# ikramanop/aligner

Hardware: AMD Instinct MI355X
Metric: GCUPS (DP cell updates/s), fill + traceback, inputs resident in HBM (higher is better)
Workload: dtype int32; 1 GPU; C5: 100000 protein pairs, lengths iid U[200,2000], core local (SimpleLocalAligner), BLOSUM62, del 11 / ext 2, seed 0xA11C0005; pairs=100000, cells=121325988939, pairs_ok_rank0=100000, pairs_repaired_or_refilled_rank0=65570

## Files before the change

aligner_amd/csrc/aln_fast.h:

```cpp
#pragma once

__device__ __forceinline__ int v_max3(int a, int b, int c)
{
    int d;
    asm("v_max3_i32 %0, %1, %2, %3" : "=v"(d) : "v"(a), "v"(b), "v"(c));
    return d;
}
__device__ __forceinline__ int v_tform(int key)
{
    int d;
    asm("v_and_or_b32 %0, %1, -4, 2" : "=v"(d) : "v"(key));
    return d;
}
__device__ __forceinline__ int v_add3_m1(int a, int b)
{
    int d;
    asm("v_add3_u32 %0, %1, %2, -1" : "=v"(d) : "v"(a), "v"(b));
    return d;
}
__device__ __forceinline__ int v_pack11(int t, int kterm)
{
    int d;
    asm("v_lshl_add_u32 %0, %1, 11, %2" : "=v"(d) : "v"(t), "s"(kterm));
    return d;
}
#define ALN_CELL_ASM(BYTE)                                                                                    \
    asm("v_add_u32_sdwa %0, %8, sext(%9) dst_sel:DWORD dst_unused:UNUSED_PAD src0_sel:DWORD src1_sel:" BYTE "\n\t" \
        "v_add_u32 %1, %5, %7\n\t"                                                                            \
        "v_add3_u32 %2, %6, %7, -1\n\t"                                                                       \
        "v_max3_i32 %3, %1, %2, %0\n\t"                                                                       \
        "v_and_or_b32 %4, %3, -4, 2"                                                                          \
        : "=&v"(c), "=&v"(a), "=&v"(b), "=&v"(key), "=v"(nt)                                                  \
        : "v"(top), "v"(left), "v"(negp), "v"(diag), "v"(pw))
template <int B>
__device__ __forceinline__ void v_cell(int top, int left, int negp, int diag, uint32_t pw, int &key, int &nt)
{
    int a, b, c;
    if constexpr (B == 0) ALN_CELL_ASM("BYTE_0");
    else if constexpr (B == 1) ALN_CELL_ASM("BYTE_1");
    else if constexpr (B == 2) ALN_CELL_ASM("BYTE_2");
    else ALN_CELL_ASM("BYTE_3");
}
#undef ALN_CELL_ASM

template <int RP> struct ProfWordP;
template <> struct ProfWordP<8> { using T = uint2; };
template <> struct ProfWordP<4> { using T = uint32_t; };
template <> struct ProfWordP<2> { using T = uint16_t; };
template <> struct ProfWordP<1> { using T = uint8_t; };
template <int R> struct ProfWord {
    static constexpr int RP = R > 4 ? 8 : R > 2 ? 4 : R;
    using T = typename ProfWordP<RP>::T;
};

template <int R>
__device__ __forceinline__ uint32_t prof_word(const typename ProfWord<R>::T &pw, int r)
{
    if constexpr (R > 4) return r < 4 ? pw.x : pw.y;
    else return (uint32_t)pw;
}
template <int R>
__device__ __forceinline__ int prof_byte(const typename ProfWord<R>::T &pw, int r)
{
    if constexpr (R > 4) return (int)(int8_t)(((r < 4 ? pw.x : pw.y) >> (8 * (r & 3))) & 0xff);
    else return (int)(int8_t)(((uint32_t)pw >> (8 * r)) & 0xff);
}

__device__ __forceinline__ int shr1_i(int old, int v) { return __builtin_amdgcn_update_dpp(old, v, 0x138, 0xf, 0xf, false); }

typedef __attribute__((address_space(3))) uint8_t aln_lds_u8;
typedef __attribute__((address_space(3))) int aln_lds_i32;
__device__ __forceinline__ void qring_put(uint32_t ring, uint32_t c, uint32_t code)
{
    const uint32_t i = c & 127u;
    *(aln_lds_u8 *)(uintptr_t)(ring + i) = (uint8_t)code;
    if (i < 64u) *(aln_lds_u8 *)(uintptr_t)(ring + 128u + i) = (uint8_t)code;
}
__device__ __forceinline__ int qring_get(uint32_t addr) { return (int)*(const aln_lds_u8 *)(uintptr_t)addr; }
__device__ __forceinline__ void bring_put(uint32_t addr, int v) { *(aln_lds_i32 *)(uintptr_t)addr = v; }
__device__ __forceinline__ int bring_get(uint32_t addr) { return *(const aln_lds_i32 *)(uintptr_t)addr; }

__device__ __forceinline__ void granule_store(uint32_t *p, int v)
{
    __hip_atomic_store(p, (uint32_t)v, __ATOMIC_RELAXED, __HIP_MEMORY_SCOPE_AGENT);
}
__device__ __forceinline__ uint32_t granule_load(const uint32_t *p)
{
    return __hip_atomic_load(p, __ATOMIC_RELAXED, __HIP_MEMORY_SCOPE_AGENT);
}

#include "aln_single_unit.inc"

#define ALN_RING 4096u

struct FastIn {
    int lane;
    uint32_t N, M;
    const uint8_t *q, *t;
    const int *S;
    uint32_t cols;
    uint8_t *prof;
    uint32_t qring;
    uint32_t brow_ring;
    int nd4, ne4;
    uint32_t *dirw;
    unsigned long long *brow_in, *brow_out;
    uint8_t *advice, *zrow;
    int *ckpt;
    bool hazard;
    bool adv_any;
    bool store_dirs;
    bool wt_dirs;
    bool pwm;
    const uint32_t *pwm_words;
    uint32_t ck_stop;
    int ck_mode;
    uint32_t last_flip;
    uint16_t *qo_pad;
    int *bring;
    const uint32_t *gin;
    uint32_t *gout;
    uint32_t lds_scratch;
    uint32_t *ring_in, *ring_out;
    uint32_t *abort_flag;
    uint32_t strip_rows, strip_q16;
    uint32_t tag_base;
    uint32_t fair;
    uint32_t ck_last;
};

struct FastOut {
    int bv;
    uint32_t by, bx;
    int corner;
    bool repaired, brow_bad, aborted;
    uint32_t ck_slot;
    uint32_t c_out;
};

template <int SEM>
__device__ __forceinline__ bool better_i(int v, uint32_t y, uint32_t x, int bv, uint32_t by, uint32_t bx)
{
    if (v > bv) return true;
    if (v < bv) return false;
    if (SEM == ALN_CORE_LOCAL) return y < by || (y == by && x < bx);
    return x > bx || (x == bx && y > by);
}

__device__ __forceinline__ uint32_t uniform32(uint32_t v) { return (uint32_t)__builtin_amdgcn_readfirstlane((int)v); }
__device__ __forceinline__ uint64_t uniform64(uint64_t v)
{
    const uint32_t lo = (uint32_t)__builtin_amdgcn_readfirstlane((int)(uint32_t)v);
    const uint32_t hi = (uint32_t)__builtin_amdgcn_readfirstlane((int)(uint32_t)(v >> 32));
    return ((uint64_t)hi << 32) | lo;
}
__device__ __forceinline__ uint64_t uniform64(const void *p) { return uniform64((uint64_t)(uintptr_t)p); }

template <int SEM, int R, bool SINGLE, bool FIRST, bool LAST, bool PWM = false>
struct FastStrip {
    static constexpr int SPB = (int)aln_spb(R);
    static constexpr int RP = ProfWord<R>::RP;
    static constexpr uint32_t CHUNK = (2048u / (4u * SPB)) * (4u * SPB);
    static constexpr uint32_t STRIP_ROWS = SINGLE ? 64u * R : (uint32_t)ALN_STRIP_ROWS;
    static constexpr bool LOCAL = (SEM == ALN_CORE_LOCAL || SEM == ALN_LEGACY_LOCAL);
    static constexpr bool QRING = !SINGLE && !PWM;
    static constexpr bool BRING = QRING && !FIRST;
    static constexpr int QSHIFT = RP == 8 ? 9 : RP == 4 ? 8 : RP == 2 ? 7 : 6;
    using PW = typename ProfWord<R>::T;
    const FastIn in;
    const uint32_t strip;
    static constexpr bool last = LAST;
    const int lane;
    const uint32_t N;
    uint32_t lb, rb, yb;
    uint32_t chunk0;
    uint32_t cchg;
    bool zsel_on, brow_bad, aborted;
    int Tl[R], rbv[R];
    int hdiag, bottom, qoff, inchunk, qchunk, outq;
    uint32_t advchunk, dw;
    PW pw;
    const uint8_t *prow;
    uint32_t qaddr;
    uint32_t baddr;

    const uint8_t *qo_lane;
    int *bring;
    int qv, top0v;
    uint32_t gpre;
    static constexpr bool GLOBAL_ASM = (SEM == ALN_CORE_GLOBAL);
    static constexpr bool ASMPATH = SINGLE && (SEM == ALN_CORE_LOCAL || SEM == ALN_CORE_GLOBAL) && (R == 1 || R == 2) && !(FIRST && LAST);
    int twov;
    PW pw1;
    uint32_t qv2, qv3, gA, gB;
    bool insteady;
    bool ring_staged;

    __device__ __forceinline__ FastStrip(const FastIn &i, uint32_t s)
        : in(i), strip(s), lane(i.lane), N(i.N), cchg(0), brow_bad(false), aborted(false) {}

    uint32_t psel_lo, psel_hi;
    __device__ __forceinline__ PW pwm_select(uint32_t w4) const
    {
        if constexpr (R > 4) return make_uint2(__builtin_amdgcn_perm(w4, w4, psel_lo), __builtin_amdgcn_perm(w4, w4, psel_hi));
        else return (PW)__builtin_amdgcn_perm(w4, w4, psel_lo);
    }

    __device__ __forceinline__ int fetch_above(uint32_t xi)
    {
        const uint32_t want = in.tag_base | (strip - 1u);
        const unsigned long long *p = in.brow_in + xi + 1;
        unsigned long long g = 0;
        uint32_t spins = 0;
        for (;;) {
            if (xi < N) g = __hip_atomic_load(p, __ATOMIC_RELAXED, __HIP_MEMORY_SCOPE_AGENT);
            if (__all(xi >= N || (uint32_t)(g >> 32) == want)) break;
            __builtin_amdgcn_s_sleep(8);
            if (++spins > (1u << 17)) { aborted = true; break; }
        }
        return (xi < N) ? (int)(uint32_t)g : 2;
    }
    __device__ __forceinline__ void flush_below(uint32_t k, uint32_t beyond)
    {
        const uint32_t x = k - 126u + (uint32_t)lane;
        if (x - 1u < N && x > beyond) {
            unsigned long long *p = in.brow_out + x;
            if (FIRST && SEM == ALN_CORE_LOCAL && in.ck_mode == 2) {
                if ((int)(uint32_t)__hip_atomic_load(p, __ATOMIC_RELAXED, __HIP_MEMORY_SCOPE_AGENT) != outq) cchg = x;
            } else
                __hip_atomic_store(p, ((unsigned long long)(in.tag_base | strip) << 32) | (uint32_t)outq, __ATOMIC_RELAXED, __HIP_MEMORY_SCOPE_AGENT);
        }
    }
    __device__ __forceinline__ void flush_tail(uint32_t ksteps)
    {
        const uint32_t kb_last = ((ksteps - 1u) / 64u) * 64u;
        flush_below(ksteps, kb_last >= 64u ? kb_last - 63u : 0u);
    }

    __device__ __forceinline__ void fair_prio()
    {
        const uint32_t slice = (uint32_t)(wall_clock64() >> (in.fair >> 8));
        if ((slice + (in.fair & 255u)) % 3u == 0u) __builtin_amdgcn_s_setprio(0);
        else __builtin_amdgcn_s_setprio(1);
    }

    template <bool MASKED>
    __device__ __forceinline__ void step(const uint32_t k, const int kk)
    {
        if ((k & 63u) == 0) {
            const uint32_t xi = k + (uint32_t)lane;
            if (!SINGLE && in.fair) fair_prio();
            if (!SINGLE && !LAST && k >= 64u) flush_below(k, 0u);
            if (BRING) {
                bring_put(in.brow_ring + 4u + 4u * (uint32_t)lane, fetch_above(xi + 1u));
                baddr = in.brow_ring + 4u;
            } else if (!FIRST && !SINGLE) inchunk = fetch_above(xi);
            if (SEM == ALN_CORE_LOCAL && FIRST && in.hazard) advchunk = (xi < N) ? in.advice[xi + 1] : 0u;
            if (!SINGLE && PWM) qchunk = (xi + 1 < N) ? (int)in.pwm_words[xi + 1] : 0;
            if (QRING) {
                qring_put(in.qring, xi + 2, (xi + 2 < N) ? (uint32_t)in.q[xi + 2] : 0u);
                qaddr = in.qring + ((k + 2u - (uint32_t)lane) & 127u);
            }
        }
        const int sel = (int)(k & 63u);
        int top0;
        if (FIRST) top0 = LOCAL ? 2 : ((k + 1 == N) ? 2 + (int)(N + 1) * in.nd4 : 2 + (int)(k + 1) * in.nd4);
        else if (SINGLE || BRING) top0 = top0v;
        else top0 = __builtin_amdgcn_readlane(inchunk, sel);
        const int topIn = shr1_i(top0, bottom);
        if (SINGLE && !FIRST) top0v = bring[(k + 1) & 127u];
        if (BRING) top0v = bring_get(baddr + 4u * (uint32_t)kk);
        const uint32_t adv = (SEM == ALN_CORE_LOCAL && FIRST) ? (uint32_t)__builtin_amdgcn_readlane((int)advchunk, sel) : 0u;
        const PW pwc = pw;
        if constexpr (SINGLE) {
            pw = *reinterpret_cast<const PW *>(prow + qv);
            qv = *reinterpret_cast<const uint16_t *>(qo_lane + 2 * (k + 2));
        } else if constexpr (QRING) {
            pw = *reinterpret_cast<const PW *>(prow + ((uint32_t)qv << QSHIFT));
            qv = qring_get(qaddr + (uint32_t)kk);
        } else {
            qoff = shr1_i(__builtin_amdgcn_readlane(qchunk, sel), qoff);
            pw = pwm_select((uint32_t)qoff);
        }
        static_assert(CHUNK == 2048u, "the tracker's chunks start at multiples of 2048 steps");
        const uint32_t kc = k & 2047u;
        const int kterm = (SEM == ALN_CORE_LOCAL) ? (int)(2047u - kc) : (int)kc;
        const uint32_t xm1 = k - (uint32_t)lane;
        if (!MASKED || xm1 < N) {
            int top = topIn, diag = hdiag;
            int cmpv = 2;
            if (SEM == ALN_CORE_LOCAL && FIRST) {
                const int l0 = __builtin_amdgcn_readfirstlane(((k == 0) || (adv != 0)) ? 2 : 1);
                asm("v_writelane_b32 %0, %1, 0" : "+v"(cmpv) : "s"(l0));
            }
            bool zr = (topIn == cmpv);
#pragma unroll
            for (int r = 0; r < R; ++r) {
                int negp;
                if (SEM == ALN_CORE_LOCAL) negp = zr ? in.nd4 : in.ne4;
                else if (SEM == ALN_CORE_GLOBAL) negp = (r == 0 && FIRST && lane == 0 && k == 0) ? in.nd4 : in.ne4;
                else negp = in.nd4;
                int key, nt;
                if (SEM == ALN_LEGACY_LOCAL) {
                    const int c = diag + prof_byte<R>(pwc, r);
                    key = max(v_max3(top + negp, v_add3_m1(Tl[r], negp), c), 3);
                    nt = v_tform(key);
                } else {
                    const uint32_t w32 = prof_word<R>(pwc, r);
                    switch (r & 3) {
                    case 0: v_cell<0>(top, Tl[r], negp, diag, w32, key, nt); break;
                    case 1: v_cell<1>(top, Tl[r], negp, diag, w32, key, nt); break;
                    case 2: v_cell<2>(top, Tl[r], negp, diag, w32, key, nt); break;
                    default: v_cell<3>(top, Tl[r], negp, diag, w32, key, nt); break;
                    }
                }
                uint32_t stored = (uint32_t)key;
                if (SEM == ALN_CORE_LOCAL) {
                    zr = (nt == 2);
                    stored = max((uint32_t)key, 3u);
                }
                dw = __builtin_amdgcn_alignbit(stored, dw, 2);
                if (LOCAL) rbv[r] = max(rbv[r], v_pack11(nt, kterm));
                diag = Tl[r];
                Tl[r] = nt;
                top = nt;
            }
            hdiag = topIn;
            bottom = Tl[R - 1];
        }
        if (!LAST) outq = __builtin_amdgcn_update_dpp(bottom, outq, 0x130, 0xf, 0xf, false);
    }

    __device__ __forceinline__ void publish(const uint32_t k)
    {
        const uint32_t c = k - 63u;
        const uint32_t col = c - 63u + (uint32_t)lane;
        const bool mine = lane >= 48 && col < N;
        if (in.ring_out) {
            uint32_t *slot = in.ring_out + (col & (ALN_RING - 1u));
            uint32_t spins = 0;
            while (__any(mine && __hip_atomic_load(slot, __ATOMIC_RELAXED, __HIP_MEMORY_SCOPE_WORKGROUP) != 0)) {
                __builtin_amdgcn_s_sleep(1);
                if (++spins > (1u << 22)) { aborted = true; break; }
            }
            if (mine) __hip_atomic_store(slot, (uint32_t)outq, __ATOMIC_RELAXED, __HIP_MEMORY_SCOPE_WORKGROUP);
            return;
        }
        if (mine) granule_store(in.gout + col, outq);
    }

    __device__ __forceinline__ void stage_boundary16(const uint32_t j)
    {
        const uint32_t col = 16u * j + (uint32_t)lane;
        const bool need = lane < 16 && col < N;
        if (in.ring_in) {
            uint32_t *slot = in.ring_in + (col & (ALN_RING - 1u));
            uint32_t g = 0, spins = 0;
            for (;;) {
                if (need) g = __hip_atomic_load(slot, __ATOMIC_RELAXED, __HIP_MEMORY_SCOPE_WORKGROUP);
                if (__all(!need || g != 0)) break;
                __builtin_amdgcn_s_sleep(1);
                ++spins;
                if (spins > (1u << 22) ||
                    ((spins & 1023u) == 0 && __hip_atomic_load(in.abort_flag, __ATOMIC_RELAXED, __HIP_MEMORY_SCOPE_AGENT) != 0)) {
                    if (lane == 0) __hip_atomic_store(in.abort_flag, 1u, __ATOMIC_RELAXED, __HIP_MEMORY_SCOPE_AGENT);
                    aborted = true;
                    break;
                }
            }
            if (need) __hip_atomic_store(slot, 0u, __ATOMIC_RELAXED, __HIP_MEMORY_SCOPE_WORKGROUP);
            if (lane < 16) bring[col & 127u] = need ? (int)g : 2;
            return;
        }
        uint32_t g = gpre;
        uint32_t spins = 0;
        while (!__all(!need || g != 0)) {
            __builtin_amdgcn_s_sleep(1);
            if (need) g = granule_load(in.gin + col);
            ++spins;
            if (spins > (1u << 22) ||
                ((spins & 1023u) == 0 && __hip_atomic_load(in.abort_flag, __ATOMIC_RELAXED, __HIP_MEMORY_SCOPE_AGENT) != 0)) {
                if (lane == 0) __hip_atomic_store(in.abort_flag, 1u, __ATOMIC_RELAXED, __HIP_MEMORY_SCOPE_AGENT);
                aborted = true;
                break;
            }
        }
        if (lane < 16) bring[col & 127u] = need ? (int)g : 2;
        const uint32_t ncol = col + 16u;
        gpre = (lane < 16 && ncol < N) ? granule_load(in.gin + ncol) : 0u;
    }

    __device__ __forceinline__ void store_zdw(uint32_t block)
    {
        if (SEM == ALN_CORE_LOCAL && zsel_on && (uint32_t)lane == lb) {
            if (SINGLE) reinterpret_cast<uint32_t *>(in.zrow)[block] = dw;
            else
                __hip_atomic_store(reinterpret_cast<unsigned long long *>(in.zrow) + block, ((unsigned long long)(in.tag_base | strip) << 32) | dw,
                                   __ATOMIC_RELAXED, __HIP_MEMORY_SCOPE_AGENT);
        }
    }

    __device__ __forceinline__ void steady_enter(const uint32_t k)
    {
        pw1 = *reinterpret_cast<const PW *>(prow + qv);
        qv2 = *reinterpret_cast<const uint16_t *>(qo_lane + 2 * (k + 2));
        qv3 = *reinterpret_cast<const uint16_t *>(qo_lane + 2 * (k + 3));
        gA = 0; gB = 0;
        if (!FIRST && !in.ring_in) {
            const uint32_t *src = in.gin + k + ((16u - (uint32_t)lane) & 15u);
            const uint32_t g0 = granule_load(src), g1 = granule_load(src + 16);
            if ((k >> 4) & 1u) { gB = g0; gA = g1; } else { gA = g0; gB = g1; }
        }
        insteady = true;
        ring_staged = true;
    }
    __device__ __forceinline__ void steady_leave(const uint32_t k)
    {
        qv = *reinterpret_cast<const uint16_t *>(qo_lane + 2 * (k + 1));
        if (!FIRST) { gpre = 0; stage_boundary16(k >> 4); top0v = bring[k & 127u]; }
        if (FIRST && SEM == ALN_CORE_LOCAL && in.hazard) {
            const uint32_t xi = (k & ~63u) + (uint32_t)lane;
            advchunk = (xi < N) ? in.advice[xi + 1] : 0u;
        }
        insteady = false;
    }
    template <bool MASKED>
    __device__ __forceinline__ void steady_run(const uint32_t kb, const uint32_t kb_end)
    {
        uint32_t ku = uniform32(kb * SPB);
        const uint32_t kend = uniform32(kb_end * SPB);
        uint32_t qop = (uint32_t)(uintptr_t)qo_lane + 2u * ku;
        const uint32_t prow32 = (uint32_t)(uintptr_t)prow;
        int kt = (int)uniform32(GLOBAL_ASM ? (uint32_t)(16 * in.nd4) : 2032u - (ku & 2047u));
        int G = (GLOBAL_ASM && FIRST) ? 2 + (int)(ku + ((16u - (uint32_t)lane) & 15u) + 1u) * in.nd4 : 2;
        int X1, O1, np, ta, tb, c0, c1, k0, p0, u0, u1;
        uint64_t um;
        uint32_t P0 = (uint32_t)pw, P1 = (uint32_t)pw1, P2, P3, Q0, Q1, Q2 = qv2, Q3 = qv3, la, w0, w1, w2, w3, st, spin;
        uint32_t vsrc = 4u * (ku + ((16u - (uint32_t)lane) & 15u));
        uint32_t vpub = 4u * (ku + (uint32_t)lane - 111u);
        uint32_t vdir = (kb >> 2) * 1024u + (uint32_t)lane * 16u;
        uint32_t vz = 4u * kb;
        const uint32_t vzero = 0;
        uint32_t amode = uniform32(in.ring_in ? 1u : 0u), pmode = uniform32(in.ring_out ? 1u : 0u);
        asm volatile("" : "+s"(amode), "+s"(pmode));
        const uint32_t vrmask = 4u * ALN_RING - 1u;
        const uint32_t vrbin = in.ring_in ? (uint32_t)(uintptr_t)in.ring_in : in.lds_scratch;
        const uint32_t vrbout = in.ring_out ? (uint32_t)(uintptr_t)in.ring_out : in.lds_scratch + 256u;
        uint32_t vrin = in.ring_in ? (vrbin | (vsrc & vrmask)) : vrbin;
        uint32_t vrout = in.ring_out ? (vrbout | (vpub & vrmask)) : vrbout + 4u * (uint32_t)lane;
        uint32_t astep = uniform32(in.ring_in ? 64u : 0u), pstep = uniform32(in.ring_out ? 64u : 0u);
        asm volatile("" : "+s"(astep), "+s"(pstep));
        uint64_t em = (ku >= 63u ? ~0ull : ((2ull << ku) - 1ull)) & (ku >= N ? (ku - N + 1u >= 64u ? 0ull : (~0ull << (ku - N + 1u))) : ~0ull), et;
        em = uniform64(em);
        int krem = (int)uniform32(N - 1u - ku);
        const uint32_t n4 = uniform32(4u * N);
        uint32_t gL = (in.ring_in && ring_staged) ? (uint32_t)bring[(ku + ((16u - (uint32_t)lane) & 15u)) & 127u] : 0u, chk;
        ring_staged = false;
        const uint64_t m48 = uniform64(0xffff000000000000ull), zmask = uniform64(zsel_on ? (1ull << lb) : 0ull);
        const uint32_t sdirs = uniform32(in.store_dirs ? 1u : 0u);
        uint8_t *dbase = reinterpret_cast<uint8_t *>(in.dirw) + (size_t)strip * (size_t)aln_uniform_strip_bytes(N, R);
        int dummyT = 2, dummyR = INT_MIN;
        int &t0ref = (R == 1) ? dummyT : Tl[0];
        int &r1ref = (R == 1) ? dummyR : rbv[R - 1];
        const uint64_t sgin = uniform64(in.gin), sgout = uniform64(in.gout), sdbase = uniform64(dbase),
                       szbase = uniform64(in.zrow), sabort = uniform64(in.abort_flag);
#define ALN_STEADY_OPERANDS                                                                                    \
        : [T0] "+&v"(t0ref), [TL] "+&v"(Tl[R - 1]), [r0] "+&v"(rbv[0]), [r1] "+&v"(r1ref), [X0] "+&v"(hdiag),       \
          [O0] "+&v"(outq), [P0] "+&v"(P0), [P1] "+&v"(P1), [Q2] "+&v"(Q2), [Q3] "+&v"(Q3), [gA] "+&v"(gA), [gB] "+&v"(gB),  \
          [G] "+&v"(G), [qop] "+&v"(qop), [vsrc] "+&v"(vsrc), [vpub] "+&v"(vpub), [vdir] "+&v"(vdir), [vz] "+&v"(vz),       \
          [vrin] "+&v"(vrin), [vrout] "+&v"(vrout), [gL] "+&v"(gL), [chk] "=&v"(chk),                                     \
          [kt] "+&s"(kt), [ku] "+&s"(ku), [st] "=&s"(st), [spin] "=&s"(spin), [em] "+&s"(em), [et] "=&s"(et), [krem] "+&s"(krem), [w0] "=&v"(w0), [w1] "=&v"(w1), \
          [w2] "=&v"(w2), [w3] "=&v"(w3), [P2] "=&v"(P2), [P3] "=&v"(P3), [Q0] "=&v"(Q0), [Q1] "=&v"(Q1),             \
          [X1] "=&v"(X1), [O1] "=&v"(O1), [np] "=&v"(np), [ta] "=&v"(ta), [tb] "=&v"(tb), [c0] "=&v"(c0),             \
          [c1] "=&v"(c1), [k0] "=&v"(k0), [p0] "=&v"(p0), [la] "=&v"(la), [u0] "=&v"(u0), [u1] "=&v"(u1), [um] "=&s"(um)                                              \
        : [two] "v"(twov), [prow] "v"(prow32), [ne] "v"(in.ne4), [nd] "v"(in.nd4), [vzero] "v"(vzero),               \
          [kend] "s"(kend), [gin] "s"(sgin), [gout] "s"(sgout), [dbase] "s"(sdbase), [zbase] "s"(szbase),         \
          [abortp] "s"(sabort), [m48] "s"(m48), [zmask] "s"(zmask), [sdirs] "s"(sdirs), [amode] "s"(amode), [n4] "s"(n4), [astep] "s"(astep), [pstep] "s"(pstep), \
          [pmode] "s"(pmode), [vrmask] "v"(vrmask), [vrbin] "v"(vrbin), [vrbout] "v"(vrbout)                          \
        : "vcc", "scc", "memory"
#define ALN_PICK(L1F, L1M, L1L, L2F, L2M, L2L)                                                                  \
        if constexpr (R == 1) {                                                                                \
            if constexpr (FIRST) asm volatile(L1F ALN_STEADY_OPERANDS);                                        \
            else if constexpr (LAST) asm volatile(L1L ALN_STEADY_OPERANDS);                                    \
            else asm volatile(L1M ALN_STEADY_OPERANDS);                                                        \
        } else {                                                                                               \
            if constexpr (FIRST) asm volatile(L2F ALN_STEADY_OPERANDS);                                        \
            else if constexpr (LAST) asm volatile(L2L ALN_STEADY_OPERANDS);                                    \
            else asm volatile(L2M ALN_STEADY_OPERANDS);                                                        \
        }
        if constexpr (MASKED) {
            static_assert(!FIRST, "strip 0 runs its ends in C++ (its first column takes del, and nothing waits on its start)");
            if constexpr (GLOBAL_ASM) { ALN_PICK(ALN_GMASKED_ASM_R1_MID, ALN_GMASKED_ASM_R1_MID, ALN_GMASKED_ASM_R1_LAST, ALN_GMASKED_ASM_R2_MID, ALN_GMASKED_ASM_R2_MID, ALN_GMASKED_ASM_R2_LAST) }
            else { ALN_PICK(ALN_MASKED_ASM_R1_MID, ALN_MASKED_ASM_R1_MID, ALN_MASKED_ASM_R1_LAST, ALN_MASKED_ASM_R2_MID, ALN_MASKED_ASM_R2_MID, ALN_MASKED_ASM_R2_LAST) }
        } else if constexpr (GLOBAL_ASM) {
            ALN_PICK(ALN_GSTEADY_ASM_R1_FIRST, ALN_GSTEADY_ASM_R1_MID, ALN_GSTEADY_ASM_R1_LAST, ALN_GSTEADY_ASM_R2_FIRST, ALN_GSTEADY_ASM_R2_MID, ALN_GSTEADY_ASM_R2_LAST)
        } else {
            ALN_PICK(ALN_STEADY_ASM_R1_FIRST, ALN_STEADY_ASM_R1_MID, ALN_STEADY_ASM_R1_LAST, ALN_STEADY_ASM_R2_FIRST, ALN_STEADY_ASM_R2_MID, ALN_STEADY_ASM_R2_LAST)
        }
#undef ALN_PICK
#undef ALN_STEADY_OPERANDS
        pw = (PW)P0; pw1 = (PW)P1; qv2 = Q2; qv3 = Q3;
        bottom = Tl[R - 1];
        if (st != 0) {
            if (lane == 0) __hip_atomic_store(in.abort_flag, 1u, __ATOMIC_RELAXED, __HIP_MEMORY_SCOPE_AGENT);
            aborted = true;
        }
    }
    __device__ __forceinline__ uint32_t advice_free_until(const uint32_t kb, const uint32_t kb_end)
    {
        const uint32_t k_end = kb_end * SPB;
        for (uint32_t k = kb * SPB; k < k_end; k += 1024u) {
            uint32_t any = 0;
            const uint32_t x0 = k + 16u * (uint32_t)lane;
#pragma unroll
            for (int i = 0; i < 16; ++i) any |= (x0 + i < N) ? (uint32_t)in.advice[x0 + i + 1] : 0u;
            const uint64_t m = __ballot(any != 0);
            if (m) {
                const uint32_t kq = ((k + 16u * (uint32_t)__builtin_ctzll(m)) / (4u * SPB)) * 4u;
                return kq < kb_end ? kq : kb_end;
            }
        }
        return kb_end;
    }

    template <bool MASKED>
    __device__ __forceinline__ void quad(uint4 *dirq, const uint32_t kb)
    {
        uint4 v = make_uint4(0, 0, 0, 0);
#pragma unroll 1
        for (uint32_t j = 0; j < 4; ++j) {
            const uint32_t k0 = (FIRST || !SINGLE) ? (uint32_t)__builtin_amdgcn_readfirstlane((int)((kb + j) * SPB)) : (kb + j) * SPB;
            if (SINGLE && !FIRST && ((k0 + SPB) & 15u) == 0) stage_boundary16((k0 + SPB) >> 4);
#pragma unroll
            for (int kk = 0; kk < SPB; ++kk) step<MASKED>(k0 + kk, kk);
            if constexpr (QRING) qaddr += (uint32_t)SPB;
            if constexpr (BRING) baddr += 4u * (uint32_t)SPB;
            if (SINGLE && !LAST && k0 + SPB >= 64u && ((k0 + SPB) & 15u) == 0) publish(k0 + SPB - 1);
            store_zdw(kb + j);
            if (j == 0) v.x = dw;
            else if (j == 1) v.y = dw;
            else if (j == 2) v.z = dw;
            else v.w = dw;
        }
        if (in.store_dirs) {
            uint4 *p = dirq + (size_t)(kb >> 2) * 64;
            if (!SINGLE && in.wt_dirs) {
                typedef uint32_t u32x4 __attribute__((ext_vector_type(4)));
                const u32x4 vv = {v.x, v.y, v.z, v.w};
                asm volatile("global_store_dwordx4 %0, %1, off sc0 sc1" :: "v"(p), "v"(vv) : "memory");
            } else *p = v;
        }
    }

    __device__ __forceinline__ void fold(FastOut &o, uint32_t base)
    {
#pragma unroll
        for (int r = 0; r < R; ++r) {
            const int v = rbv[r];
            const uint32_t y = yb + 1 + r;
            if (v != INT_MIN && y <= in.M) {
                const int t = v >> 11;
                const uint32_t kk = (uint32_t)v & 2047u;
                const uint32_t k = base + ((SEM == ALN_CORE_LOCAL) ? 2047u - kk : kk);
                const uint32_t x = k - (uint32_t)lane + 1;
                if (o.bx == 0 || better_i<SEM>(t, y, x, o.bv, o.by, o.bx)) { o.bv = t; o.by = y; o.bx = x; }
            }
            rbv[r] = INT_MIN;
        }
    }

    __device__ __forceinline__ void fold_saved(FastOut &o, uint32_t slot)
    {
        const int *base = in.ckpt + slot * (18 * 64) + lane;
#pragma unroll
        for (int r = 0; r < R; ++r) {
            const int v = base[(2 * r + 1) * 64];
            const uint32_t y = yb + 1 + r;
            if (v != INT_MIN && y <= in.M) {
                const int t = v >> 11;
                const uint32_t kk = (uint32_t)v & 2047u;
                const uint32_t k = (SEM == ALN_CORE_LOCAL) ? 2047u - kk : kk;
                const uint32_t x = k - (uint32_t)lane + 1;
                if (o.bx == 0 || better_i<SEM>(t, y, x, o.bv, o.by, o.bx)) { o.bv = t; o.by = y; o.bx = x; }
            }
        }
    }

    __device__ __forceinline__ bool checkpoint(uint32_t slot, bool save, const FastOut &o, bool &tracker, bool &stale)
    {
        int *base = in.ckpt + slot * (18 * 64) + lane;
        bool same = true;
#pragma unroll
        for (int r = 0; r < R; ++r) {
            if (save) { base[(2 * r) * 64] = Tl[r]; base[(2 * r + 1) * 64] = rbv[r]; }
            else {
                same = same && base[(2 * r) * 64] == Tl[r];
                const int old = base[(2 * r + 1) * 64];
                if (old != rbv[r]) {
                    tracker = true;
                    const uint32_t y = yb + 1 + r;
                    if (old != INT_MIN && y <= in.M) {
                        const uint32_t kk = (uint32_t)old & 2047u;
                        const uint32_t k = (SEM == ALN_CORE_LOCAL) ? 2047u - kk : kk;
                        if ((old >> 11) == o.bv && y == o.by && k - (uint32_t)lane + 1 == o.bx) stale = true;
                    }
                }
            }
        }
        if (save) { base[16 * 64] = hdiag; base[17 * 64] = bottom; }
        else same = same && base[16 * 64] == hdiag && base[17 * 64] == bottom;
        return same;
    }

    __device__ __forceinline__ FastOut run(FastOut o)
    {
        const uint32_t M = in.M;
        const uint32_t y0 = strip * (SINGLE ? STRIP_ROWS : in.strip_rows);
        const uint32_t rows = min(M - y0, (uint32_t)(64 * R));
        const uint32_t L = (rows + R - 1) / R;
        const uint32_t nsteps = (SINGLE && !LAST) ? N + 63 : N + L - 1;
        yb = y0 + (uint32_t)lane * R;
        lb = (rows - 1) / R; rb = (rows - 1) % R;
        zsel_on = (SEM == ALN_CORE_LOCAL) && LAST && in.hazard;
        prow = in.prof + lane * RP;

        int tc[R];
#pragma unroll
        for (int r = 0; r < R; ++r) {
            const uint32_t y = yb + 1 + r;
            tc[r] = (y <= M) ? (int)in.t[y - 1] * (int)in.cols : 0;
            Tl[r] = LOCAL ? 2 : (y == M ? 2 + (int)(M + 1) * in.nd4 : 2 + (int)y * in.nd4);
            rbv[r] = INT_MIN;
        }
        psel_lo = 0; psel_hi = 0;
#pragma unroll
        for (int r = 0; r < R; ++r) {
            const uint32_t y = yb + 1 + r;
            const uint32_t code = (y <= M) ? (uint32_t)in.t[y - 1] & 3u : 0u;
            if (r < 4) psel_lo |= code << (8 * r); else psel_hi |= code << (8 * (r - 4));
        }
        for (uint32_t c = 0; c < (PWM ? 0u : in.cols); ++c) {
            uint32_t lo = 0, hi = 0;
#pragma unroll
            for (int r = 0; r < R; ++r) {
                const uint32_t bte = (uint32_t)(4 * in.S[tc[r] + c] - 2) & 0xffu;
                if (r < 4) lo |= bte << (8 * r); else hi |= bte << (8 * (r - 4));
            }
            uint8_t *dst = in.prof + c * (64 * RP) + lane * RP;
            if constexpr (RP == 8) *reinterpret_cast<uint2 *>(dst) = make_uint2(lo, hi);
            else if constexpr (RP == 4) *reinterpret_cast<uint32_t *>(dst) = lo;
            else if constexpr (RP == 2) *reinterpret_cast<uint16_t *>(dst) = (uint16_t)lo;
            else *dst = (uint8_t)lo;
        }
        hdiag = LOCAL || yb == 0 ? 2 : 2 + (int)yb * in.nd4;
        bottom = Tl[R - 1];
        inchunk = 2; qchunk = 0; advchunk = 0; dw = 0; outq = 0; qv = 0; top0v = 2;
        twov = (FIRST && lane == 0) ? 1 : 2;
        pw1 = PW{}; qv2 = 0; qv3 = 0; gA = 0; gB = 0; insteady = false; ring_staged = false;
        if constexpr (SINGLE) {
            qo_lane = reinterpret_cast<const uint8_t *>(in.qo_pad + 63 - lane);
            bring = in.bring;
            gpre = (!FIRST && !in.ring_in && lane < 16 && (uint32_t)lane < N) ? granule_load(in.gin + lane) : 0u;
            if (!FIRST) { stage_boundary16(0); top0v = bring[0]; }
            qoff = *reinterpret_cast<const uint16_t *>(qo_lane);
            qv = *reinterpret_cast<const uint16_t *>(qo_lane + 2);
        } else {
            qoff = (lane == 0) ? (PWM ? (int)in.pwm_words[0] : (int)in.q[0] * (64 * RP)) : 0;
            if constexpr (QRING) {
                const uint32_t c1 = 1u - (uint32_t)lane;
                qv = (c1 < N) ? (int)in.q[c1] : 0;
                qring_put(in.qring, c1, (uint32_t)qv);
                qaddr = in.qring + ((2u - (uint32_t)lane) & 127u);
                baddr = in.brow_ring + 4u;
                if constexpr (BRING) top0v = __builtin_amdgcn_readfirstlane(fetch_above(lane == 0 ? 0u : 0xffffffffu));
            }
        }
        if (!SINGLE && PWM) pw = pwm_select((uint32_t)qoff);
        else pw = *reinterpret_cast<const PW *>(prow + qoff);

        uint4 *dirq = reinterpret_cast<uint4 *>(in.dirw) +
                      (size_t)strip * (SINGLE ? (size_t)(aln_uniform_strip_bytes(N, R) / 16) : (size_t)in.strip_q16) + lane;
        const uint32_t nkb = aln_strip_blocks(nsteps, SPB);
        const uint32_t kb_steady0 = min(nkb, ((uint32_t)((63 + SPB) / SPB) + 3u) & ~3u);
        uint32_t kb_steady1 = max(kb_steady0, min(nkb, (N / (4 * SPB)) * 4u));
        if (ASMPATH && GLOBAL_ASM && FIRST && kb_steady1 * SPB >= N && kb_steady1 >= kb_steady0 + 4u) kb_steady1 -= 4u;
        const bool cks = SINGLE && SEM == ALN_CORE_LOCAL && in.ck_mode != 0 && in.ck_stop != 0;
        const bool ckmode = cks || (FIRST && !SINGLE && SEM == ALN_CORE_LOCAL && in.ck_mode != 0);
        uint32_t next_ck = cks ? in.ck_stop : ckmode ? ((ALN_CK_FIRST + 4u * SPB - 1u) / (4u * SPB)) * (4u * SPB) : 0xffffffffu, slot = 0, chunk_base = 0;
        chunk0 = 0;
        uint32_t kb = 0;
        while (kb < nkb) {
            uint32_t seg_end = min(nkb, (chunk_base + CHUNK) / SPB);
            if (next_ck != 0xffffffffu) seg_end = min(seg_end, next_ck / SPB);
            const uint32_t e0 = min(kb_steady0, seg_end), e1 = min(kb_steady1, seg_end);
            if constexpr (ASMPATH && !FIRST) {
                if (!aborted) {
                    if (!insteady) steady_enter(kb * SPB);
                    if (kb < e0) { steady_run<true>(kb, e0); kb = e0; }
                    if (kb < e1 && !aborted) { steady_run<false>(kb, e1); kb = e1; }
                    if (kb < seg_end && !aborted) { steady_run<true>(kb, seg_end); kb = seg_end; }
                }
                if (aborted) { o.aborted = true; return o; }
            }
            for (; kb < e0; kb += 4) quad<true>(dirq, kb);
            if constexpr (ASMPATH) {
                while (kb < e1 && !aborted) {
                    uint32_t kb_to = e1;
                    if (FIRST && in.adv_any) {
                        kb_to = advice_free_until(kb, e1);
                        if (kb_to == kb) {
                            if (insteady) steady_leave(kb * SPB);
                            quad<false>(dirq, kb);
                            kb += 4;
                            continue;
                        }
                    }
                    if (!insteady) steady_enter(kb * SPB);
                    steady_run<false>(kb, kb_to);
                    kb = kb_to;
                }
                if (aborted) { o.aborted = true; return o; }
                if (FIRST && insteady && kb >= kb_steady1) steady_leave(kb * SPB);
            }
            for (; kb < e1; kb += 4) quad<false>(dirq, kb);
            for (; kb < seg_end; kb += 4) quad<true>(dirq, kb);
            if (cks && kb < nkb && kb * SPB == next_ck) {
                bool tracker = false, stale = false;
                if (in.ck_mode == 1) { checkpoint(0, true, o, tracker, stale); next_ck = 0xffffffffu; }
                else {
                    o.repaired = __all(checkpoint(0, false, o, tracker, stale));
                    o.aborted = o.aborted || aborted;
                    return o;
                }
            } else if (ckmode && kb < nkb && kb * SPB == next_ck) {
                bool tracker = false, stale = false;
                if (in.ck_mode == 1) checkpoint(slot, true, o, tracker, stale);
                else if (__all(checkpoint(slot, false, o, tracker, stale)) && in.last_flip <= next_ck) {
                    if (!__any(stale)) {
                        if (__any(tracker)) fold(o, 0);
                        o.repaired = true;
                        o.ck_slot = slot;
                        if (!LAST) flush_tail(kb * SPB);
                        o.c_out = __any(cchg != 0u) ? 1u : 0u;
                    }
                    return o;
                }
                ++slot;
                const uint32_t lim = (in.ck_mode == 2 && in.last_flip <= 512u) ? 512u : in.ck_last;
                next_ck = next_ck < lim ? next_ck * 2u : 0xffffffffu;
                if (in.ck_mode == 2 && next_ck == 0xffffffffu) return o;
            }
            if (kb * SPB == chunk_base + CHUNK) {
                if (LOCAL) fold(o, chunk_base);
                chunk_base += CHUNK;
                chunk0 = uniform32(chunk_base);
            }
        }
        if (SINGLE && !LAST && !(ASMPATH && !FIRST)) publish(nkb * SPB - 1);
        if (!SINGLE && !LAST && !(ckmode && in.ck_mode == 2)) flush_tail(nkb * SPB);
        o.brow_bad = o.brow_bad || brow_bad;
        o.aborted = o.aborted || aborted;
        if (ckmode && in.ck_mode == 2) return o;
        if (LOCAL) fold(o, chunk_base);
        if (last) {
            int hb = Tl[0];
#pragma unroll
            for (int r = 1; r < R; ++r) if ((uint32_t)r == rb) hb = Tl[r];
            o.corner = __builtin_amdgcn_readlane(hb, (int)lb);
        }
        return o;
    }
};

#define ALN_STRIP_CASE(RR, FIRSTV, LASTV) case RR: { FastStrip<SEM, RR, false, FIRSTV, LASTV, PWM> f(in, s); return f.run(o); }
template <int SEM, bool PWM, bool FIRSTV>
__device__ __forceinline__ FastOut fast_strip_of(const FastIn &in, FastOut o, uint32_t s, bool last, int R)
{
// ... 33 lines not shown
```

aligner_amd/csrc/aln_kernels.hip:

```cpp
#include <hip/hip_runtime.h>
#include <float.h>
#include <limits.h>
#include <math.h>

#include "aln_device.h"

#define ALN_PART_GENERIC 1
#define ALN_PART_FAST_CL 2
#define ALN_PART_FAST_REST 4
#define ALN_PART_FAST_CL_SOLO 32
#define ALN_PART_FAST_REST_SOLO 64
#define ALN_PART_SINGLE 8
#define ALN_PART_TB 16
#ifndef ALN_TU
#define ALN_TU 127
#endif

namespace {

constexpr int D_TOP = 0, D_LEFT = 1, D_DIAG = 2, D_BEG = 3;

template <typename SC> struct ScOps;

template <> struct ScOps<int> {
// ... 2441 lines not shown
        const uint32_t q = kb >> 2, rel = q - q_lo;
        uint32_t word = lds3[((min(rel, q_n - 1u) * 64u + lane) << 2) + (kb & 3u)];
        if (__builtin_expect(rel >= q_n, 0)) word = wbase[(((uint64_t)q * 64u + lane) << 2) + (kb & 3u)];
        return word;
    };
    if (threadIdx.x == 0) walk_in_strip(fetch, y0, lgR, d.N, global, cy, cx, steps, ops);
}

extern "C" __global__ __launch_bounds__(1024) void aln_tb_single_expand_kernel(TraceArgs a, uint32_t pair)
{
    __shared__ uint32_t wsum_y[16], wsum_x[16];
    const PairDesc &d = a.descs[pair];
    const aln_pair_result &res = a.results[pair];
    if (res.status != ALN_OK || (d.layout & 0xffu) != ALN_LAYOUT_UNIFORM) return;
    const uint32_t tid = threadIdx.x, lane = tid & 63u, wave = tid >> 6;
    const uint8_t *__restrict__ q = a.seqs + d.q_off;
    const uint8_t *__restrict__ t = a.seqs + d.t_off;
    const uint32_t cap = d.N + d.M + 2;
    uint8_t *__restrict__ qa = a.tb + d.tb_off;
    uint8_t *__restrict__ ta = qa + (a.pwm ? 4ull : 1ull) * cap;
    uint32_t *__restrict__ numbered = reinterpret_cast<uint32_t *>(qa);
    const uint8_t *__restrict__ ops = a.tags + d.tag_off;
    const uint32_t len = res.aln_len - (a.pwm ? 0u : 1u);
    const uint32_t per = (len + 1023u) / 1024u;
    const uint32_t lo = min(len, tid * per), hi = min(len, lo + per);
    uint32_t dy = 0, dx = 0;
    for (uint32_t j = lo; j < hi; ++j) {
        const uint32_t tag = ops[len - 1 - j];
        dx += (tag != 2u); dy += (tag != 1u);
    }
    uint32_t sy = dy, sx = dx;
#pragma unroll
    for (int m = 1; m < 64; m <<= 1) {
        const uint32_t oy = (uint32_t)__shfl_up((int)sy, m), ox = (uint32_t)__shfl_up((int)sx, m);
        if ((int)lane >= m) { sy += oy; sx += ox; }
    }
    if (lane == 63) { wsum_y[wave] = sy; wsum_x[wave] = sx; }
    __syncthreads();
    uint32_t by = 0, bx = 0;
    for (uint32_t wv = 0; wv < wave; ++wv) { by += wsum_y[wv]; bx += wsum_x[wv]; }
    uint32_t py = res.start_y + by + sy - dy, px = res.start_x + bx + sx - dx;
    for (uint32_t j = lo; j < hi; ++j) {
        const uint32_t tag = ops[len - 1 - j];
        px += (tag != 2u); py += (tag != 1u);
        if (a.pwm) numbered[j] = (tag == 2u) ? 0u : px;
        else qa[j] = (tag == 2u) ? a.blank : q[px - 1];
        ta[j] = (tag == 1u) ? a.blank : t[py - 1];
    }
    if (tid == 0 && !a.pwm) {
        qa[len] = q[res.end_x - 1];
        ta[len] = t[res.end_y - 1];
    }
}

extern "C" __global__ __attribute__((amdgpu_flat_work_group_size(256, 256), amdgpu_num_vgpr(16))) void aln_traceback_expand_kernel(TraceArgs a)
{
    const uint32_t pair = blockIdx.x * (blockDim.x >> 6) + (threadIdx.x >> 6);
    if (pair >= a.n_pairs) return;
    constexpr int G = 2;
    const int lane = threadIdx.x & 63;
    const PairDesc &d = a.descs[pair];
    const aln_pair_result &res = a.results[pair];
    if (res.status != ALN_OK) return;
    if ((d.layout & 0xffu) == ALN_LAYOUT_UNIFORM) return;
    const uint8_t *__restrict__ q = a.seqs + d.q_off;
    const uint8_t *__restrict__ t = a.seqs + d.t_off;
    const uint32_t cap = d.N + d.M + 2;
    uint8_t *__restrict__ qa = a.tb + d.tb_off;
    uint8_t *__restrict__ ta = qa + (a.pwm ? 4ull : 1ull) * cap;
    const uint8_t *__restrict__ ops = a.tags + d.tag_off;
    uint32_t *__restrict__ numbered = reinterpret_cast<uint32_t *>(qa);
    const uint32_t len = res.aln_len - (a.pwm ? 0u : 1u);
    uint32_t base_y = (uint32_t)__builtin_amdgcn_readfirstlane((int)res.start_y);
    uint32_t base_x = (uint32_t)__builtin_amdgcn_readfirstlane((int)res.start_x);
    for (uint32_t j0 = 0; j0 < len; j0 += 64u * G) {
        uint32_t tag[G], px[G], py[G];
#pragma unroll
        for (int u = 0; u < G; ++u) {
            const uint32_t j = j0 + 64u * u + (uint32_t)lane;
            tag[u] = (j < len) ? (uint32_t)ops[len - 1 - j] : 3u;
        }
#pragma unroll
        for (int u = 0; u < G; ++u) {
            const bool fx = (tag[u] != 2u) && (tag[u] != 3u), fy = (tag[u] != 1u) && (tag[u] != 3u);
            const uint64_t bx = __ballot(fx), by = __ballot(fy);
            px[u] = base_x + __builtin_amdgcn_mbcnt_hi((uint32_t)(bx >> 32), __builtin_amdgcn_mbcnt_lo((uint32_t)bx, 0u)) + (fx ? 1u : 0u);
            py[u] = base_y + __builtin_amdgcn_mbcnt_hi((uint32_t)(by >> 32), __builtin_amdgcn_mbcnt_lo((uint32_t)by, 0u)) + (fy ? 1u : 0u);
            base_x += (uint32_t)__popcll(bx); base_y += (uint32_t)__popcll(by);
        }
        uint32_t qv[G], tv[G];
#pragma unroll
        for (int u = 0; u < G; ++u) {
            qv[u] = (tag[u] == 2u || tag[u] == 3u) ? (uint32_t)a.blank : (a.pwm ? px[u] : (uint32_t)q[px[u] - 1]);
            tv[u] = (tag[u] == 1u || tag[u] == 3u) ? (uint32_t)a.blank : (uint32_t)t[py[u] - 1];
        }
#pragma unroll
        for (int u = 0; u < G; ++u) {
            const uint32_t j = j0 + 64u * u + (uint32_t)lane;
            if (j < len) {
                if (a.pwm) numbered[j] = (tag[u] == 2u) ? 0u : px[u];
                else qa[j] = (uint8_t)qv[u];
                ta[j] = (uint8_t)tv[u];
            }
        }
    }
    if (lane == 0 && !a.pwm) {
        qa[len] = q[res.end_x - 1];
        ta[len] = t[res.end_y - 1];
    }
}

extern "C" __global__ void aln_unpack_directions_kernel(const uint8_t *dirs, const PairDesc *descs, uint32_t pair,
                                                        int semantics, uint8_t *out)
{
    const PairDesc d = descs[pair];
    const uint64_t total = (uint64_t)(d.M + 1) * (d.N + 1);
    const bool global = (semantics == ALN_CORE_GLOBAL || semantics == ALN_LEGACY_GLOBAL);
    for (uint64_t i = (uint64_t)blockIdx.x * blockDim.x + threadIdx.x; i < total; i += (uint64_t)gridDim.x * blockDim.x) {
        const uint32_t y = (uint32_t)(i / (d.N + 1)), x = (uint32_t)(i % (d.N + 1));
        out[i] = (uint8_t)dir_at(dirs, d, global, y, x);
    }
}

#endif

#define ALN_FAST_GO(...)                                                                                                   \
    do {                                                                                                                   \
        auto kern = &__VA_ARGS__;                                                                                          \
        if (lds_bytes > 64u * 1024u)                                                                                       \
            (void)hipFuncSetAttribute(reinterpret_cast<const void *>(kern), hipFuncAttributeMaxDynamicSharedMemorySize, (int)lds_bytes); \
        hipLaunchKernelGGL(kern, g, b, lds_bytes, s, *a);                                                                  \
    } while (0)
#define ALN_FAST_REST_LAUNCH(COOPV)                                                                                        \
    switch (a->semantics) {                                                                                                \
    case ALN_CORE_GLOBAL: ALN_FAST_GO(aln_fill_fast_kernel<ALN_CORE_GLOBAL, false, COOPV>); break; \
    case ALN_CORE_LOCAL: ALN_FAST_GO(aln_fill_fast_kernel<ALN_CORE_LOCAL, true, COOPV>); break;    \
    case ALN_LEGACY_GLOBAL: ALN_FAST_GO(aln_fill_fast_kernel<ALN_LEGACY_GLOBAL, false, COOPV>); break; \
    default: ALN_FAST_GO(aln_fill_fast_kernel<ALN_LEGACY_LOCAL, false, COOPV>); break;      \
    }
#if ALN_TU & ALN_PART_FAST_CL
extern "C" void aln_launch_fill_fast_cl(const FillArgs *a, uint32_t grid, uint32_t lds_bytes, hipStream_t s)
{
    const dim3 g(grid), b(256);
    ALN_FAST_GO(aln_fill_fast_kernel<ALN_CORE_LOCAL, false, true>);
}
#endif
#if ALN_TU & ALN_PART_FAST_CL_SOLO
extern "C" void aln_launch_fill_fast_cl_solo(const FillArgs *a, uint32_t grid, uint32_t lds_bytes, hipStream_t s)
{
    const dim3 g(grid), b(256);
    ALN_FAST_GO(aln_fill_fast_kernel<ALN_CORE_LOCAL, false, false>);
}
#endif
#if ALN_TU & ALN_PART_FAST_REST
extern "C" void aln_launch_fill_fast_rest(const FillArgs *a, uint32_t grid, uint32_t lds_bytes, hipStream_t s)
{
    const dim3 g(grid), b(256);
    ALN_FAST_REST_LAUNCH(true)
}
#endif
#if ALN_TU & ALN_PART_FAST_REST_SOLO
__device__ __forceinline__ bool lane_is_first_cell(uint32_t j, uint32_t k) { return j == 0u && k == 0u; }
template <int R>
__device__ __forceinline__ void duo_fill(const FillArgs &a, uint8_t *prof, uint16_t *qo, const uint32_t qo_stride, const int *S, const int lane,
                                         const uint32_t N, const uint32_t M, const uint8_t *q, const uint8_t *t, uint4 *dirq, const uint32_t myquads,
                                         const uint32_t nsteps, const uint32_t maxN, int &corner)
{
    constexpr int SPB = (int)aln_spb(R);
    constexpr int RP = ProfWord<R>::RP;
    using PW = typename ProfWord<R>::T;
    const uint32_t j = (uint32_t)lane & 31u, h = (uint32_t)lane >> 5;
    const int nd4 = -4 * (int)a.del, ne4 = -4 * (int)a.ext;
    uint16_t *myqo = qo + h * qo_stride;
    for (uint32_t i = j; i < maxN + 136u; i += 32u) myqo[i] = (i >= 32u && i - 32u < N) ? (uint16_t)((uint32_t)q[i - 32u] * (64u * RP)) : (uint16_t)0;
    int tc[R], Tl[R];
    const uint32_t yb = j * R;
#pragma unroll
    for (int r = 0; r < R; ++r) {
        const uint32_t y = yb + 1 + r;
        tc[r] = (y <= M) ? (int)t[y - 1] * (int)a.cols : 0;
        Tl[r] = (y == M) ? 2 + (int)(M + 1) * nd4 : 2 + (int)y * nd4;
    }
    for (uint32_t c = 0; c < a.cols; ++c) {
        uint32_t lo = 0, hi = 0;
#pragma unroll
        for (int r = 0; r < R; ++r) {
            const uint32_t bte = (uint32_t)(4 * S[tc[r] + c] - 2) & 0xffu;
            if (r < 4) lo |= bte << (8 * r); else hi |= bte << (8 * (r - 4));
        }
        uint8_t *dst = prof + c * (64 * RP) + lane * RP;
        if constexpr (RP == 8) *reinterpret_cast<uint2 *>(dst) = make_uint2(lo, hi);
        else if constexpr (RP == 4) *reinterpret_cast<uint32_t *>(dst) = lo;
        else if constexpr (RP == 2) *reinterpret_cast<uint16_t *>(dst) = (uint16_t)lo;
        else *dst = (uint8_t)lo;
    }
    __builtin_amdgcn_fence(__ATOMIC_RELEASE, "wavefront");
    __builtin_amdgcn_wave_barrier();
    const uint8_t *prow = prof + lane * RP;
    const uint16_t *qmine = myqo + 32u - j;
    int hdiag = (yb == 0) ? 2 : 2 + (int)yb * nd4;
    int bottom = Tl[R - 1];
    uint32_t dw = 0;
    PW pw = *reinterpret_cast<const PW *>(prow + qmine[0]);
    uint32_t qv = qmine[1];
    const uint32_t nkb = ((nsteps + SPB - 1) / SPB + 3u) & ~3u;
    for (uint32_t kb = 0; kb < nkb; kb += 4) {
        uint4 v = make_uint4(0, 0, 0, 0);
#pragma unroll 1
        for (uint32_t b4 = 0; b4 < 4; ++b4) {
            const uint32_t k0 = (uint32_t)__builtin_amdgcn_readfirstlane((int)((kb + b4) * SPB));
#pragma unroll
            for (int kk = 0; kk < SPB; ++kk) {
                const uint32_t k = k0 + (uint32_t)kk;
                const int top0 = (k + 1 == N) ? 2 + (int)(N + 1) * nd4 : 2 + (int)(k + 1) * nd4;
                int topIn = shr1_i(top0, bottom);
                topIn = (j == 0) ? top0 : topIn;
                const PW pwc = pw;
                pw = *reinterpret_cast<const PW *>(prow + qv);
                qv = qmine[k + 2];
                const uint32_t xm1 = k - j;
                if (xm1 < N) {
                    int top = topIn, diag = hdiag;
#pragma unroll
                    for (int r = 0; r < R; ++r) {
                        const int negp = (r == 0 && lane_is_first_cell(j, k)) ? nd4 : ne4;
                        int key, nt;
                        const uint32_t w32 = prof_word<R>(pwc, r);
                        switch (r & 3) {
                        case 0: v_cell<0>(top, Tl[r], negp, diag, w32, key, nt); break;
                        case 1: v_cell<1>(top, Tl[r], negp, diag, w32, key, nt); break;
                        case 2: v_cell<2>(top, Tl[r], negp, diag, w32, key, nt); break;
                        default: v_cell<3>(top, Tl[r], negp, diag, w32, key, nt); break;
                        }
                        dw = __builtin_amdgcn_alignbit((uint32_t)key, dw, 2);
                        diag = Tl[r];
                        Tl[r] = nt;
                        top = nt;
                    }
                    hdiag = topIn;
                    bottom = Tl[R - 1];
                }
            }
            if (b4 == 0) v.x = dw;
            else if (b4 == 1) v.y = dw;
            else if (b4 == 2) v.z = dw;
            else v.w = dw;
        }
        if (a.store_dirs && (kb >> 2) < myquads) dirq[(size_t)(kb >> 2) * 64] = v;
    }
    const uint32_t rb = (M - 1u) % R;
    int hb = Tl[0];
#pragma unroll
    for (int r = 1; r < R; ++r) if ((uint32_t)r == rb) hb = Tl[r];
    corner = hb;
}

extern "C" __global__ __attribute__((amdgpu_flat_work_group_size(256, 256), amdgpu_waves_per_eu(3, 3)))
void aln_fill_duo_kernel(FillArgs a)
{
    extern __shared__ __attribute__((aligned(16))) unsigned char smem[];
    int *S = reinterpret_cast<int *>(smem);
    const int *gm = reinterpret_cast<const int *>(a.matrix);
    for (uint32_t i = threadIdx.x; i < a.rows * a.cols; i += blockDim.x) S[i] = gm[i];
    __syncthreads();
    const int lane = threadIdx.x & 63;
    const uint32_t wv = threadIdx.x >> 6;
    uint8_t *wbase = smem + ((a.rows * a.cols * 4u + 15u) & ~15u) + wv * (a.prof_stride + 4u * a.duo_qo);
    uint8_t *prof = wbase;
    uint16_t *qo = reinterpret_cast<uint16_t *>(wbase + a.prof_stride);
    const uint32_t h = (uint32_t)lane >> 5;
    uint32_t run_left = 0, run_pos = 0;
    const uint32_t n_items = (a.n_pairs + 1u) / 2u, claim = a.claim ? a.claim : 1u;
    for (;;) {
        if (run_left == 0u) {
            unsigned long long v = 0;
            if (lane == 0) v = __hip_atomic_fetch_add(reinterpret_cast<unsigned long long *>(a.counter + 4), (unsigned long long)claim, __ATOMIC_RELAXED, __HIP_MEMORY_SCOPE_AGENT);
            const uint32_t f = (uint32_t)__builtin_amdgcn_readfirstlane((int)(uint32_t)v);
            if (f >= n_items) break;
            run_pos = f; run_left = min(claim, n_items - f);
        }
        const uint32_t item = run_pos++;
        --run_left;
        const uint32_t qpos = 2u * item + h;
        const bool have = qpos < a.n_pairs;
        const uint32_t pair = have ? a.order[qpos] : 0u;
        const PairDesc &d = a.descs[pair];
        int st = have ? d.status : ALN_ERR_INVALID_ARGUMENT;
        uint32_t N = have ? d.N : 0u, M = have ? d.M : 0u;
        const uint8_t *q = a.seqs + d.q_off, *t = a.seqs + d.t_off;
        if (st == ALN_OK) {
            uint32_t worst_q = 0, worst_t = 0;
            for (uint32_t i = (uint32_t)lane & 31u; i < N; i += 32u) worst_q = max(worst_q, (uint32_t)q[i]);
            for (uint32_t i = (uint32_t)lane & 31u; i < M; i += 32u) worst_t = max(worst_t, (uint32_t)t[i]);
            const uint64_t badm = __ballot(worst_q >= a.cols || worst_t >= a.rows);
            if ((badm >> (32u * h)) & 0xffffffffull) st = ALN_ERR_CODE_OUT_OF_RANGE;
        }
        const bool ok = st == ALN_OK;
        if (!ok) { N = 0; M = 0; }
        const uint32_t Rl = ok ? (M + 31u) / 32u : 1u;
        uint32_t R = max((uint32_t)__builtin_amdgcn_readlane((int)Rl, 0), (uint32_t)__builtin_amdgcn_readlane((int)Rl, 32));
        const uint32_t L = ok ? (M + R - 1u) / R : 0u;
        const uint32_t st_l = ok ? N + L - 1u : 0u;
        const uint32_t nsteps = max((uint32_t)__builtin_amdgcn_readlane((int)st_l, 0), (uint32_t)__builtin_amdgcn_readlane((int)st_l, 32));
        const uint32_t maxN = max((uint32_t)__builtin_amdgcn_readlane((int)N, 0), (uint32_t)__builtin_amdgcn_readlane((int)N, 32));
        uint4 *dirq = reinterpret_cast<uint4 *>(a.dirs + d.dir_off) + ((uint32_t)lane & 31u);
        const uint32_t myquads = ok ? aln_strip_blocks(N + 63u, aln_spb(R)) / 4u : 0u;
// ... 265 lines not shown
```

Before: 2870 GCUPS.

## Skip per-cell local-best tracking until a wave-wide threshold is exceeded

In multi-strip local fill, the per-cell max/pack update of the row-best values is replaced by a per-step check: each lane takes the max of its column values, a ballot tests whether any lane reaches a wave-uniform threshold, and only then the packed best values are updated and the threshold raised via a DPP wave max. The threshold is seeded from the previous strip's best. This removes a pack-and-max from every cell's inner loop, at the cost of a ballot plus a reduction per step and a branch that fires whenever new maxima appear. Optional stats counters are compiled in only when ALN_TRACK_STATS is defined.

```diff
diff --git a/aligner_amd/csrc/aln_fast.h b/aligner_amd/csrc/aln_fast.h
--- a/aligner_amd/csrc/aln_fast.h
+++ b/aligner_amd/csrc/aln_fast.h
@@ -67,6 +67,15 @@
 }
 
 __device__ __forceinline__ int shr1_i(int old, int v) { return __builtin_amdgcn_update_dpp(old, v, 0x138, 0xf, 0xf, false); }
+__device__ __forceinline__ int wave_max_i(int v)
+{
+    v = max(v, __builtin_amdgcn_update_dpp(v, v, 0xb1, 0xf, 0xf, false));
+    v = max(v, __builtin_amdgcn_update_dpp(v, v, 0x4e, 0xf, 0xf, false));
+    v = max(v, __builtin_amdgcn_update_dpp(v, v, 0x141, 0xf, 0xf, false));
+    v = max(v, __builtin_amdgcn_update_dpp(v, v, 0x140, 0xf, 0xf, false));
+    return max(max(__builtin_amdgcn_readlane(v, 0), __builtin_amdgcn_readlane(v, 16)),
+               max(__builtin_amdgcn_readlane(v, 32), __builtin_amdgcn_readlane(v, 48)));
+}
 
 typedef __attribute__((address_space(3))) uint8_t aln_lds_u8;
 typedef __attribute__((address_space(3))) int aln_lds_i32;
@@ -92,6 +101,10 @@
 #include "aln_single_unit.inc"
 
 #define ALN_RING 4096u
+
+#ifdef ALN_TRACK_STATS
+__device__ unsigned long long aln_track_stats_dev[2];
+#endif
 
 struct FastIn {
     int lane;
@@ -163,6 +176,7 @@
     static constexpr uint32_t CHUNK = (2048u / (4u * SPB)) * (4u * SPB);
     static constexpr uint32_t STRIP_ROWS = SINGLE ? 64u * R : (uint32_t)ALN_STRIP_ROWS;
     static constexpr bool LOCAL = (SEM == ALN_CORE_LOCAL || SEM == ALN_LEGACY_LOCAL);
+    static constexpr bool THRTRK = LOCAL && !SINGLE;
     static constexpr bool QRING = !SINGLE && !PWM;
     static constexpr bool BRING = QRING && !FIRST;
     static constexpr int QSHIFT = RP == 8 ? 9 : RP == 4 ? 8 : RP == 2 ? 7 : 6;
@@ -181,6 +195,11 @@
     uint32_t advchunk, dw;
     PW pw;
     const uint8_t *prow;
+    int thr;
+    int nvalid;
+#ifdef ALN_TRACK_STATS
+    uint32_t st_steps, st_upd;
+#endif
     uint32_t qaddr;
     uint32_t baddr;
 
@@ -198,6 +217,12 @@
 
     __device__ __forceinline__ FastStrip(const FastIn &i, uint32_t s)
         : in(i), strip(s), lane(i.lane), N(i.N), cchg(0), brow_bad(false), aborted(false) {}
+#ifdef ALN_TRACK_STATS
+    __device__ __forceinline__ ~FastStrip()
+    {
+        if (THRTRK && lane == 0) { atomicAdd(&aln_track_stats_dev[0], (unsigned long long)st_steps); atomicAdd(&aln_track_stats_dev[1], (unsigned long long)st_upd); }
+    }
+#endif
 
     uint32_t psel_lo, psel_hi;
     __device__ __forceinline__ PW pwm_select(uint32_t w4) const
@@ -320,7 +345,7 @@
                     stored = max((uint32_t)key, 3u);
                 }
                 dw = __builtin_amdgcn_alignbit(stored, dw, 2);
-                if (LOCAL) rbv[r] = max(rbv[r], v_pack11(nt, kterm));
+                if (LOCAL && !THRTRK) rbv[r] = max(rbv[r], v_pack11(nt, kterm));
                 diag = Tl[r];
                 Tl[r] = nt;
                 top = nt;
@@ -328,7 +353,34 @@
             hdiag = topIn;
             bottom = Tl[R - 1];
         }
+        if constexpr (THRTRK) {
+            int m = Tl[0];
+#pragma unroll
+            for (int r = 1; r + 1 < R; r += 2) m = max(max(m, Tl[r]), Tl[r + 1]);
+            if (R % 2 == 0) m = max(m, Tl[R - 1]);
+            const bool act = !MASKED || xm1 < N;
+#ifdef ALN_TRACK_STATS
+            ++st_steps;
+#endif
+            uint64_t hit = __builtin_amdgcn_ballot_w64(m >= thr);
+            if (MASKED) hit &= __builtin_amdgcn_ballot_w64(act);
+            if (hit != 0ull) track(kterm, act);
+        }
         if (!LAST) outq = __builtin_amdgcn_update_dpp(bottom, outq, 0x130, 0xf, 0xf, false);
+    }
+
+    __device__ __forceinline__ void track(const int kterm, const bool act)
+    {
+        int mv = INT_MIN;
+#pragma unroll
+        for (int r = 0; r < R; ++r) {
+            if (act) rbv[r] = max(rbv[r], v_pack11(Tl[r], kterm));
+            if (!LAST || r < nvalid) mv = max(mv, Tl[r]);
+        }
+        thr = __builtin_amdgcn_readfirstlane(max(thr, wave_max_i(act ? mv : INT_MIN)));
+#ifdef ALN_TRACK_STATS
+        ++st_upd;
+#endif
     }
 
     __device__ __forceinline__ void publish(const uint32_t k)
@@ -623,6 +675,12 @@
         lb = (rows - 1) / R; rb = (rows - 1) % R;
         zsel_on = (SEM == ALN_CORE_LOCAL) && LAST && in.hazard;
         prow = in.prof + lane * RP;
+        nvalid = (int)min((uint32_t)R, M - min(M, yb));
+        thr = INT_MIN;
+        if (THRTRK && !FIRST) thr = __builtin_amdgcn_readfirstlane(wave_max_i(o.bx != 0 ? o.bv : INT_MIN));
+#ifdef ALN_TRACK_STATS
+        st_steps = 0; st_upd = 0;
+#endif
 
         int tc[R];
 #pragma unroll
diff --git a/aligner_amd/csrc/aln_kernels.hip b/aligner_amd/csrc/aln_kernels.hip
--- a/aligner_amd/csrc/aln_kernels.hip
+++ b/aligner_amd/csrc/aln_kernels.hip
@@ -2617,6 +2617,17 @@
     ALN_FAST_GO(aln_fill_fast_kernel<ALN_CORE_LOCAL, false, false>);
 }
 #endif
+#if defined(ALN_TRACK_STATS) && (ALN_TU & (ALN_PART_FAST_CL | ALN_PART_FAST_CL_SOLO | ALN_PART_FAST_REST | ALN_PART_FAST_REST_SOLO))
+#define ALN_TRACK_CAT2(a, b) a##b
+#define ALN_TRACK_CAT(a, b) ALN_TRACK_CAT2(a, b)
+extern "C" int ALN_TRACK_CAT(aln_debug_track_stats_, ALN_TU)(unsigned long long *out)
+{
+    const unsigned long long zero[2] = {0ull, 0ull};
+    if (hipDeviceSynchronize() != hipSuccess) return -1;
+    if (hipMemcpyFromSymbol(out, HIP_SYMBOL(aln_track_stats_dev), sizeof(zero)) != hipSuccess) return -1;
+    return hipMemcpyToSymbol(HIP_SYMBOL(aln_track_stats_dev), zero, sizeof(zero)) == hipSuccess ? 0 : -1;
+}
+#endif
 #if ALN_TU & ALN_PART_FAST_REST
 extern "C" void aln_launch_fill_fast_rest(const FillArgs *a, uint32_t grid, uint32_t lds_bytes, hipStream_t s)
 {
```

New measurement: 2842 GCUPS. No clear change (-1.0%).
